# ftl/sdrainer

Measured on AMD Instinct MI355X. Metric: IQ MSamples/s through FFT+peak+envelope, higher is better.
Workload: dtype f64

## Files before the change

### sdrainer_amd/csrc/bank.h

```cpp
#pragma once
#include <hip/hip_runtime.h>

#include <algorithm>
#include <atomic>
#include <chrono>
#include <cmath>
#include <cstdio>
#include <cstdlib>
#include <cstring>
#include <memory>
#include <mutex>
#include <string>
#include <thread>
#include <vector>

#include "../../include/sdrainer_hip.h"
#include "host/delivery.h"
#include "host/frequency_mapping.h"
#include "sdr_device.h"

namespace sdrcapi {

inline thread_local std::string g_last_error;

// ... 70 lines not shown
    DevBuf<sdr::DevPeak> dev_peaks;
    DevBuf<int> peak_counts;
    hipEvent_t done[sdr::K_COUNT] = {};
    void release()
    {
        psd.release();
        tap.release();
        tapw.release();
        tap_used.release();
        fft_ctr.release();
        fft_scratch.release();
        win_mean.release();
        cum_part.release();
        recs.release();
        raw_bits.release();
        bits.release();
        edges.release();
        edge_counts.release();
        tr_values.release();
        tr_raw.release();
        tr_deb.release();
        slots_before.release();
        cum_out.release();
        dev_peaks.release();
        peak_counts.release();
        for (auto &e : done) {
            if (e)
                (void)hipEventDestroy(e);
            e = nullptr;
        }
    }
};


enum Parts { PART_SPECTRA = 1, PART_LISTEN = 2, PART_ALL = 3 };

struct CursorPack {
    sdr::BatchCursor c[RING];
};

}

struct sdr_bank {
    template <class T>
    using DevBuf = sdrcapi::DevBuf<T>;
    using BatchSet = sdrcapi::BatchSet;
    static constexpr int N_STAGES = sdrcapi::N_STAGES, GRAPH_PHASES = sdrcapi::GRAPH_PHASES, N_GRAPHS = sdrcapi::N_GRAPHS, RING = sdrcapi::RING;

    sdr_config cfg{};
    sdr::Switches sw;
    int logn = 0;
    int hop = 0;
    int device = 0;
    hipStream_t stream[N_STAGES] = {};
    bool own_stream[N_STAGES] = {};

    int max_chunks = 0;
    int text_cap = 2048;
    int edge_cap = 0;
    int bit_words = 0;

    DevBuf<fft64::cplx> tw;
    DevBuf<unsigned char> db_tab;
    DevBuf<int32_t> tap_bins;
    DevBuf<float> window;
    bool windowed = false;
    DevBuf<float> spectrum_row;
    std::vector<BatchSet> set;
    DevBuf<sdr::BandState> band_state;
    DevBuf<sdr::ListenerSlot> slots;
    DevBuf<uint16_t> morse;
    DevBuf<uint32_t> text;
    DevBuf<uint32_t> text_frames;
    DevBuf<uint32_t> edge_pos;
    DevBuf<float> carry[2];

    std::vector<sdr::BandState> h_band_state;
    std::vector<sdr::ListenerSlot> h_slots;
    std::vector<int> n_slots;
    std::vector<int64_t> center_frequency;
    int carry_cur = 0;
    int cum_count = 0;
    int64_t total_frames = 0;
    int64_t batch_index = 0;
    int last_set = 0, last_frames = 0, last_chunks = 0, last_count0 = 0;
    int last_carry_in = 0;
    int edge_width = 0;
    int find_peaks = 1;
    bool failed = false;
    DevBuf<sdr::DropCounters> drops;
    DevBuf<sdr::BatchCursor> cursors;
    hipGraph_t graph[GRAPH_PHASES][N_GRAPHS] = {};
    hipGraphExec_t graph_exec[GRAPH_PHASES][N_GRAPHS] = {};
    hipGraphNode_t graph_cursor_node[GRAPH_PHASES] = {};
    hipEvent_t phase_done[GRAPH_PHASES][N_GRAPHS] = {};
    int64_t graph_base = 0;
    int64_t graph_replays = 0;
    bool graph_ready = false;
    int graph_frames = 0, graph_slots = 0;
    sdr::InFormat graph_fmt = sdr::InFormat::F32;
    uint64_t attach_gen = 0, graph_attach_gen = 0;
    bool graph_results_on = false;
    int graph_find_peaks = 0;
    bool defer_listen = false, listen_pending = false;
    struct PendingListen {
        int set = 0, frames = 0;
// ... 91 lines not shown
```

### sdrainer_amd/csrc/capi_bank.hip

```cpp
#include "bank.h"
#include "twiddles.h"

using namespace sdrcapi;

namespace sdr {
int set_error(int code, const char *msg) { return fail(code, msg); }
}

namespace sdrcapi {
std::unique_ptr<host::DeliveryBackend> make_results_backend(sdr_bank *b);

void resolve_profile(sdr_bank *b)
{
    for (auto &p : b->pending) {
        float ms = 0.f;
        if (hipEventElapsedTime(&ms, p.second.first, p.second.second) == hipSuccess) {
            b->prof_ms[p.first] += ms;
            b->prof_n[p.first] += 1;
        }
        (void)hipEventDestroy(p.second.first);
        (void)hipEventDestroy(p.second.second);
    }
    b->pending.clear();
}
// ... 117 lines not shown
    return SDR_OK;
}

namespace {
static int self_check_once(int device_id)
{
    constexpr int kMax = 64;
    static std::mutex mu;
    static int verdict[kMax];
    static bool done[kMax];
    static std::string message[kMax];
    if (device_id < 0 || device_id >= kMax)
        return sdr_self_check(device_id);
    std::lock_guard<std::mutex> g(mu);
    if (!done[device_id]) {
        verdict[device_id] = sdr_self_check(device_id);
        message[device_id] = g_last_error;
        done[device_id] = verdict[device_id] == SDR_OK || message[device_id].find("self-check failed") != std::string::npos;
    }
    if (verdict[device_id] != SDR_OK)
        g_last_error = message[device_id];
    return verdict[device_id];
}
}

int sdr_create(const sdr_config *cfg, sdr_bank **out)
{
    if (!cfg || !out)
        return fail(SDR_ERR_BAD_ARG, "null argument");
    if (cfg->struct_size != (int32_t)sizeof(sdr_config))
        return fail(SDR_ERR_BAD_ARG, "sdr_config.struct_size mismatch (ABI)");
    const int N = cfg->block_size;
    if (N < 512 || N > 65536 || (N & (N - 1)))
        return fail(SDR_ERR_BAD_SIZE, "block_size must be a power of two in [512, 65536]");
    if (cfg->n_bands < 1 || cfg->sample_rate < 1 || cfg->max_batch_frames < 1 || cfg->max_listeners < 0 ||
        cfg->max_peaks < 1)
        return fail(SDR_ERR_BAD_ARG, "non-positive geometry");
    if (cfg->edge_width < 0 || N - 2 * cfg->edge_width < 10)
        return fail(SDR_ERR_BAD_ARG, "edge_width leaves fewer than 10 bins: the reference's windowSize would be 0 (NaN)");
    if (!sdr::hop_valid(cfg->hop, N))
        return fail(SDR_ERR_BAD_ARG, "hop must be 0 (= block_size) or a power of two with block_size / 16 <= hop <= block_size and hop >= 32");
    int ndev = 0;
    HIP_TRY(hipGetDeviceCount(&ndev));
    if (cfg->device_id < 0 || cfg->device_id >= ndev)
        return fail(SDR_ERR_BAD_ARG, "device_id out of range");
    HIP_TRY(hipSetDevice(cfg->device_id));

    sdr_bank *b = new sdr_bank();
    b->cfg = *cfg;
    b->hop = sdr::effective_hop(cfg->hop, N);
    b->sw = sdr::read_switches();
    b->device = cfg->device_id;
    b->logn = ilog2(N);
    b->edge_width = cfg->edge_width;
    b->find_peaks = cfg->find_peaks;
    const size_t B = (size_t)cfg->n_bands, L = (size_t)cfg->max_listeners;
    b->max_chunks = cfg->max_batch_frames / SDR_CUMULATION_SIZE + 2;
    b->edge_cap = cfg->max_batch_frames < 8192 ? cfg->max_batch_frames : 8192;
    b->bit_words = (cfg->max_batch_frames + 63) / 64;

#define ALLOC(buf, count)                                                                              \
    do {                                                                                               \
        hipError_t _e = (buf).alloc(count);                                                            \
        if (_e != hipSuccess) {                                                                        \
            sdr_destroy(b);                                                                            \
            return fail(SDR_ERR_HIP, std::string("hipMalloc " #buf ": ") + hipGetErrorString(_e));     \
        }                                                                                              \
    } while (0)

    for (int s = 1; s < N_STAGES && !b->sw.no_overlap; s++) {
        hipError_t e = hipStreamCreateWithFlags(&b->stream[s], hipStreamNonBlocking);
        if (e != hipSuccess) {
            sdr_destroy(b);
            return fail(SDR_ERR_HIP, "hipStreamCreate failed");
        }
        b->own_stream[s] = true;
    }
    if (sdr::may_use_matrix_pipe(b->sw, N)) {
        const int sc = self_check_once(cfg->device_id);
        if (sc != SDR_OK) {
            sdr_destroy(b);
            return sc;
        }
    }
    {
        std::vector<double> wre, wim;
        fft64::radix2_factors(N, wre, wim);
        const size_t ntw = (size_t)sdr::twiddle_count(b->logn);
        std::vector<fft64::cplx> h(ntw);
        sdr::build_twiddles(b->logn, wre.data(), wim.data(), h.data());
        ALLOC(b->tw, h.size());
        hipError_t e = hipMemcpy(b->tw.p, h.data(), h.size() * sizeof(fft64::cplx), hipMemcpyHostToDevice);
        std::vector<unsigned char> tab(gomath::kDbTabBytes);
        gomath::build_db_tables(b->logn, tab.data());
        ALLOC(b->db_tab, tab.size());
        if (e == hipSuccess)
            e = hipMemcpy(b->db_tab.p, tab.data(), tab.size(), hipMemcpyHostToDevice);
        if (e != hipSuccess) {
            sdr_destroy(b);
            return fail(SDR_ERR_HIP, "twiddle / table upload failed");
        }
    }
    b->res_backend = make_results_backend(b);
    b->results.reset(new host::Delivery(b->res_backend.get(), RING, GRAPH_PHASES * RING));
    b->set.reserve((size_t)RING + (size_t)GRAPH_PHASES * RING);
    b->set.resize(RING);
// ... 389 lines not shown
```

### sdrainer_amd/csrc/capi_process.hip

```cpp
#include <string>

#include "bank.h"

using namespace sdrcapi;

namespace sdrcapi {

constexpr int PUT_SLOTS = 16, PUT_BINS = 128;
struct SlotPack {
    int32_t n;
    int32_t index[PUT_SLOTS];
    sdr::ListenerSlot slot[PUT_SLOTS];
};
struct BinPack {
    int32_t n;
    int32_t index[PUT_BINS], bin[PUT_BINS];
};
__global__ void k_put_slots(sdr::ListenerSlot *slots, SlotPack p)
{
    constexpr int W = sizeof(sdr::ListenerSlot) / 4;
    static_assert(sizeof(sdr::ListenerSlot) % 4 == 0, "word copy");
    for (int i = threadIdx.x; i < p.n * W; i += blockDim.x)
        reinterpret_cast<uint32_t *>(slots + p.index[i / W])[i % W] = reinterpret_cast<const uint32_t *>(&p.slot[i / W])[i % W];
}
// ... 33 lines not shown
        HIP_TRY(hipGetLastError());
    }
    b->late_attached.clear();
    return SDR_OK;
}


int process_device_impl(sdr_bank *b, const void *iq_dev, int n_frames, size_t in_stride, sdr::InFormat fmt)
{
    if (b->failed)
        return fail(SDR_ERR_STATE, "an earlier process call failed half way; destroy the bank");
    if (b->graph_ready)
        return fail(SDR_ERR_STATE, "a graph is captured: process through sdr_graph_launch, or sdr_graph_release first");
    if (b->listen_pending)
        return fail(SDR_ERR_STATE, "the previous batch still waits for its listen half (sdr_process_listen)");
    const int rc = process_device_body(b, iq_dev, n_frames, in_stride, -1, -1, b->defer_listen ? PART_SPECTRA : PART_ALL, fmt);
    if (rc == SDR_ERR_HIP)
        b->failed = true;
    return rc;
}

int process_device_body(sdr_bank *b, const void *iq_dev, int n_frames, size_t in_stride, int capture_k, int capture_stage, int parts,
                        sdr::InFormat fmt)
{
    const bool cap = capture_k >= 0;
    const bool do_spectra = (parts & PART_SPECTRA) != 0, do_listen = (parts & PART_LISTEN) != 0;
    if (!do_spectra)
        n_frames = b->pend.frames;
    const sdr::BatchCursor *cur = cap ? b->cursors.p + capture_k : nullptr;
    const sdr_config &c = b->cfg;
    if (n_frames <= 0)
        return SDR_OK;
    struct DisarmOnExit {
        ~DisarmOnExit() { sdr::t_done_event = nullptr; }
    } disarm_on_exit;
    if (n_frames > c.max_batch_frames)
        return fail(SDR_ERR_BAD_ARG, "n_frames exceeds max_batch_frames");
    HIP_TRY(hipSetDevice(b->device));
    if (!cap) {
        const int frc = flush_late_attached(b);
        if (frc)
            return frc;
    }
    const int B = c.n_bands, N = c.block_size, stride = c.max_batch_frames;
    const sdr::NoiseGeom ng = b->noise_geom();
    const int si = cap ? RING + capture_k : do_spectra ? (int)(b->batch_index % RING) : b->pend.set;
    const int64_t first_frame = do_spectra ? b->total_frames : b->pend.first_frame;
    BatchSet &S = b->set[si];
    host::ResultSet &RS = b->results->set(si);
    int max_slots = 0;
    for (int i = 0; i < B; i++)
        max_slots = std::max(max_slots, b->n_slots[i]);
    const int count0 = b->cum_count;
    const sdr::BatchPlan P = sdr::plan_batch(b->sw, sdr::BatchGeometry{B, N, stride, b->max_chunks}, n_frames, count0, cap, max_slots, b->windowed);
    const int *plan = P.stream;
    const sdr::CumGeom cg{N, stride, n_frames, count0, b->max_chunks};
#define SDR_ON(k) (!cap || (capture_stage == G_THRESHOLDS ? (k) == sdr::K_THRESHOLDS : (plan[k] == capture_stage && (k) != sdr::K_THRESHOLDS)))
#if defined(SDR_DIAG)
#define SDR_LAUNCH(id, call) \
    do {                     \
        if (!(b->sw.diag_skip >> (id) & 1) && SDR_ON(id)) \
            HIP_TRY(call);   \
    } while (0)
#else
#define SDR_LAUNCH(id, call)  \
    do {                      \
        if (SDR_ON(id))       \
            HIP_TRY(call);    \
    } while (0)
#endif
    auto stream_of = [&](int k) { return b->stream[plan[k]]; };
    auto after = [&](int k, int dep) -> int {
        if (stream_of(k) != stream_of(dep) && !cap)
            HIP_TRY(hipStreamWaitEvent(stream_of(k), S.done[dep], 0));
        return SDR_OK;
    };
#define SDR_AFTER(k, dep)          \
    do {                           \
        int _rc = after((k), (dep)); \
        if (_rc)                   \
            return _rc;            \
    } while (0)
#define SDR_ARM(k) (sdr::t_done_event = cap ? nullptr : S.done[k])
#define SDR_DONE(k)                                                                                   \
    do {                                                                                              \
        if (sdr::t_done_event && !cap) {                                                              \
            sdr::t_done_event = nullptr;                                                              \
            HIP_TRY(hipEventRecord(S.done[k], stream_of(k)));                                         \
        }                                                                                             \
    } while (0)

    if (do_spectra) {
    if (b->results_on && !cap) {
        const int prc = b->results->park(si);
        if (prc)
            return prc;
    }
    {
        static const int launch_order[] = {sdr::K_WINDOW_MEANS, sdr::K_NOISE_STATS, sdr::K_THRESHOLDS, sdr::K_LISTEN_GATHER,
                                           sdr::K_LISTEN_DECODE, sdr::K_CUMULATE,   sdr::K_FIND_PEAKS};
        int last_on[N_STAGES];
        for (int &l : last_on)
            l = -1;
        for (int k : launch_order)
            last_on[plan[k]] = k;
        for (int st = 0; st < N_STAGES; st++) {
            const int k = last_on[st];
            if (k < 0 || st == plan[sdr::K_FFT])
                continue;
            if (cap)
                continue;
            if (hipEventQuery(S.done[k]) == hipSuccess)
                continue;
            HIP_TRY(hipStreamWaitEvent(stream_of(sdr::K_FFT), S.done[k], 0));
        }
    }
    if (cap && SDR_ON(sdr::K_FFT) && capture_k % RING == 0)
        HIP_TRY(launch_set_cursors(b->cursors.p + capture_k, CursorPack{}, stream_of(sdr::K_FFT)));
    {
        ProfScope ps(b, sdr::K_FFT, stream_of(sdr::K_FFT));
        SDR_ARM(sdr::K_FFT);
        sdr::FftTap tap{b->tap_bins.p, S.tap.p, max_slots, c.max_listeners};
        tap.wide = S.tapw.p;
        tap.used = S.tap_used.p;
        tap.steal = S.fft_ctr.p;
        tap.scratch = S.fft_scratch.p;
        tap.window = b->windowed ? b->window.p : nullptr;
        SDR_LAUNCH(sdr::K_FFT, sdr::launch_fft(b->logn, P.fft, fmt, iq_dev, cur, b->tw.p, S.psd.p, n_frames, B, in_stride, b->hop, stride, tap,
                                               stream_of(sdr::K_FFT)));
    }
    SDR_DONE(sdr::K_FFT);

    SDR_AFTER(sdr::K_WINDOW_MEANS, sdr::K_FFT);
    {
        ProfScope ps(b, sdr::K_WINDOW_MEANS, stream_of(sdr::K_WINDOW_MEANS));
        SDR_ARM(sdr::K_WINDOW_MEANS);
        if (P.noise_scan) {
            SDR_LAUNCH(sdr::K_WINDOW_MEANS, sdr::launch_psd_scan(S.psd.p, S.recs.p, S.cum_out.p, S.cum_part.p, cur, ng, cg, P.n_slots, B, P.bound_done,
                                                                 P.scan_parts, P.force_exact, stream_of(sdr::K_WINDOW_MEANS)));
        } else {
            SDR_LAUNCH(sdr::K_WINDOW_MEANS, sdr::launch_window_means(S.psd.p, S.win_mean.p, ng, n_frames, B, stride, P.wm_wpb,
                                                                     stream_of(sdr::K_WINDOW_MEANS)));
        }
    }
    SDR_DONE(sdr::K_WINDOW_MEANS);
    SDR_AFTER(sdr::K_NOISE_STATS, sdr::K_WINDOW_MEANS);
    {
        ProfScope ps(b, sdr::K_NOISE_STATS, stream_of(sdr::K_NOISE_STATS));
        SDR_ARM(sdr::K_NOISE_STATS);
        if (!P.noise_scan)
            SDR_LAUNCH(sdr::K_NOISE_STATS, sdr::launch_noise_stats(S.psd.p, S.win_mean.p, S.recs.p, ng, n_frames, B, stride, P.var_mfma,
                                                                   stream_of(sdr::K_NOISE_STATS)));
    }
    SDR_DONE(sdr::K_NOISE_STATS);
    SDR_AFTER(sdr::K_THRESHOLDS, sdr::K_NOISE_STATS);
    {
        ProfScope ps(b, sdr::K_THRESHOLDS, stream_of(sdr::K_THRESHOLDS));
        SDR_ARM(sdr::K_THRESHOLDS);
        SDR_LAUNCH(sdr::K_THRESHOLDS, sdr::launch_thresholds(S.recs.p, b->band_state.p, n_frames, B, stride,
                                                             stream_of(sdr::K_THRESHOLDS)));
    }
    SDR_DONE(sdr::K_THRESHOLDS);
    }

    sdr::ListenGeom lg;
    lg.n = N;
    lg.stride = stride;
    lg.max_listeners = c.max_listeners;
    lg.text_cap = b->text_cap;
    lg.edge_cap = b->edge_cap;
    lg.bit_words = b->bit_words;
    lg.trace = c.trace;
    lg.frame_base = (uint32_t)first_frame;
    if (do_listen) {
    SDR_AFTER(sdr::K_LISTEN_GATHER, sdr::K_THRESHOLDS);
    SDR_AFTER(sdr::K_LISTEN_GATHER, sdr::K_FFT);
    if (!cap && b->slots_put) {
        if (hipEventQuery(b->slots_put_ev) == hipSuccess)
            b->slots_put = false;
        else if (plan[sdr::K_LISTEN_GATHER] != S_LISTEN)
            HIP_TRY(hipStreamWaitEvent(stream_of(sdr::K_LISTEN_GATHER), b->slots_put_ev, 0));
    }
    SDR_ARM(sdr::K_LISTEN_GATHER);
    if (max_slots > 0) {
        ProfScope ps(b, sdr::K_LISTEN_GATHER, stream_of(sdr::K_LISTEN_GATHER));
        SDR_LAUNCH(sdr::K_LISTEN_GATHER, sdr::launch_listen_gather(S.tap.p, S.psd.p, S.recs.p, b->slots.p, b->db_tab.p, S.raw_bits.p, S.tr_values.p,
                                                                   S.tr_raw.p, cur, lg, n_frames, max_slots, B,
                                                                   stream_of(sdr::K_LISTEN_GATHER)));
    }
    SDR_DONE(sdr::K_LISTEN_GATHER);
    SDR_AFTER(sdr::K_LISTEN_DECODE, sdr::K_LISTEN_GATHER);
    if (c.trace && max_slots > 0 && SDR_ON(sdr::K_LISTEN_DECODE))
        HIP_TRY(hipMemcpyAsync(S.slots_before.p, b->slots.p, sizeof(sdr::ListenerSlot) * (size_t)B * (size_t)c.max_listeners,
                               hipMemcpyDeviceToDevice, stream_of(sdr::K_LISTEN_DECODE)));
    if (!b->results_on)
        SDR_ARM(sdr::K_LISTEN_DECODE);
    if (max_slots > 0) {
        ProfScope ps(b, sdr::K_LISTEN_DECODE, stream_of(sdr::K_LISTEN_DECODE));
        SDR_LAUNCH(sdr::K_LISTEN_DECODE, sdr::launch_listen_decode(b->slots.p, b->morse.p, S.raw_bits.p, S.bits.p, b->text.p,
                                                                   b->text_frames.p, S.edges.p, S.edge_counts.p, S.tr_deb.p, b->drops.p, cur,
                                                                   lg, n_frames, B, b->edge_pos.p, c.max_batch_frames, stream_of(sdr::K_LISTEN_DECODE)));
    }
    if (b->results_on && SDR_ON(sdr::K_LISTEN_DECODE)) {
        SDR_ARM(sdr::K_LISTEN_DECODE);
        HIP_TRY(sdr::launch_pack_listen(b->slots.p, S.edges.p, S.edge_counts.p, b->text.p, b->text_frames.p, b->drops.p, b->res_layout, max_slots, B,
                                        RS.block, stream_of(sdr::K_LISTEN_DECODE)));
        if (!cap)
            HIP_TRY(hipEventRecord(static_cast<hipEvent_t>(RS.ev_listen), stream_of(sdr::K_LISTEN_DECODE)));
    }
    SDR_DONE(sdr::K_LISTEN_DECODE);
    }
    if (!do_spectra) {
        b->results->complete(si, max_slots, b->pend.batch);
        b->listen_pending = false;
        return SDR_OK;
    }

    const int n_chunks = P.n_chunks;
    SDR_AFTER(sdr::K_CUMULATE, sdr::K_FFT);
    if (P.bound_done)
        SDR_AFTER(sdr::K_CUMULATE, sdr::K_WINDOW_MEANS);
    {
        ProfScope ps(b, sdr::K_CUMULATE, stream_of(sdr::K_CUMULATE));
        SDR_ARM(sdr::K_CUMULATE);
        SDR_LAUNCH(sdr::K_CUMULATE, sdr::launch_cumulate(S.psd.p, b->db_tab.p, b->carry[0].p, b->carry[1].p, b->carry_cur, S.cum_out.p, S.cum_part.p,
                                                         cur, cg, P.n_slots, B, P.bound, P.bound_done, P.scan_parts, stream_of(sdr::K_CUMULATE)));
    }
    SDR_DONE(sdr::K_CUMULATE);
    SDR_AFTER(sdr::K_FIND_PEAKS, sdr::K_CUMULATE);
    if (!b->results_on)
        SDR_ARM(sdr::K_FIND_PEAKS);
    if (b->find_peaks && n_chunks > 0) {
        SDR_AFTER(sdr::K_FIND_PEAKS, sdr::K_THRESHOLDS);
        ProfScope ps(b, sdr::K_FIND_PEAKS, stream_of(sdr::K_FIND_PEAKS));
        sdr::PeakGeom pg{N, stride, count0, b->max_chunks, c.max_peaks};
        sdr::FftTap wide_tap{nullptr, nullptr, max_slots, c.max_listeners};
        if (P.fft.wide_tap) {
            wide_tap.wide = S.tapw.p;
            wide_tap.used = S.tap_used.p;
        }
        SDR_LAUNCH(sdr::K_FIND_PEAKS, sdr::launch_find_peaks(S.cum_out.p, S.psd.p, b->db_tab.p, b->carry[0].p, b->carry[1].p, b->carry_cur, S.recs.p,
                                                             S.dev_peaks.p, S.peak_counts.p, cur, pg, n_frames, n_chunks, B, P.refine, wide_tap,
                                                             stream_of(sdr::K_FIND_PEAKS)));
    }
    if (b->results_on && SDR_ON(sdr::K_FIND_PEAKS)) {
        SDR_ARM(sdr::K_FIND_PEAKS);
        HIP_TRY(sdr::launch_pack_peaks(S.dev_peaks.p, S.peak_counts.p, cur, b->res_layout, b->find_peaks, n_frames, n_chunks, B,
                                       RS.block, stream_of(sdr::K_FIND_PEAKS)));
        if (!cap) {
            HIP_TRY(hipEventRecord(static_cast<hipEvent_t>(RS.ev_peaks), stream_of(sdr::K_FIND_PEAKS)));
            host::BatchMeta m;
            m.batch = b->batch_index;
            m.first_frame = b->total_frames;
            m.frames = n_frames;
            m.chunks = n_chunks;
            m.count0 = count0;
            m.slots = do_listen ? max_slots : 0;
            {
                std::lock_guard<std::mutex> guard(b->center_mu);
                m.center = b->center_frequency;
            }
            b->results->publish(si, std::move(m), do_listen);
        }
    }
    SDR_DONE(sdr::K_FIND_PEAKS);
#undef SDR_AFTER
#undef SDR_DONE
#undef SDR_ARM
#undef SDR_LAUNCH
#undef SDR_ON

    if (cap)
        return SDR_OK;
    b->last_carry_in = b->carry_cur;
    if (P.new_count != 0)
        b->carry_cur ^= 1;
    b->cum_count = P.new_count;
    b->last_set = si;
    b->last_frames = n_frames;
// ... 306 lines not shown
```

### sdrainer_amd/csrc/host/batch_plan.h

```cpp
#pragma once
#include <cstdint>
#include <cstdlib>
#include <cstring>

#include "../../../include/sdrainer_hip.h"

namespace sdr {

enum KernelId {
    K_FFT = 0, K_WINDOW_MEANS, K_NOISE_STATS, K_THRESHOLDS, K_LISTEN_GATHER, K_CUMULATE, K_FIND_PEAKS, K_LISTEN_DECODE,
    K_COUNT
};
enum Stage { S_FFT = 0, S_NOISE, S_LISTEN, S_PEAKS, N_STAGES };

constexpr int kR32MaxTap = 512;

struct Switches {
    bool noise_scan = true;
    int force_exact = 0;
    int fft_r32 = -1;
    int fft_fpw = 0;
    int cum_bound = -1;
    int refine_wide = -1;
    int var_mfma = -1;
    int wm_wpb = 0;
    int fft2p_group_mb = -1;
    bool no_overlap = false;
    bool graph_debug = false;
    int diag_skip = 0;
    int diag_plan[K_COUNT] = {-1, -1, -1, -1, -1, -1, -1, -1};
};

inline int tri_state(const char *e)
{
    if (!e)
        return -1;
    const int v = atoi(e);
    return v >= 0 ? (v != 0 ? 1 : 0) : -1;
}

inline Switches read_switches()
{
    Switches s;
    const char *e;
    if ((e = getenv("SDR_NOISE_PATH")))
        s.noise_scan = strcmp(e, "chains") != 0;
    if ((e = getenv("SDR_NOISE_FORCE_EXACT")))
        s.force_exact = atoi(e);
    if ((e = getenv("SDR_FFT_R32")))
        s.fft_r32 = atoi(e) ? 1 : 0;
    if ((e = getenv("SDR_FFT_FPW"))) {
        const int v = atoi(e);
        s.fft_fpw = v < 1 ? 1 : (v > 64 ? 64 : v);
    }
    s.cum_bound = tri_state(getenv("SDR_CUM_BOUND"));
    s.refine_wide = tri_state(getenv("SDR_REFINE_WIDE"));
    s.var_mfma = tri_state(getenv("SDR_VAR_MFMA"));
    if ((e = getenv("SDR_FFT2P_GROUP_MB")))
        s.fft2p_group_mb = atoi(e) >= 0 ? atoi(e) : -1;
    if ((e = getenv("SDR_WM_WPB")))
        s.wm_wpb = atoi(e) > 0 ? atoi(e) : 0;
    e = getenv("SDR_NO_OVERLAP");
    s.no_overlap = e && e[0] == '1';
    s.graph_debug = getenv("SDR_GRAPH_DEBUG") != nullptr;
#if defined(SDR_DIAG)
    if ((e = getenv("SDR_DIAG_SKIP")))
        s.diag_skip = atoi(e);
    if ((e = getenv("SDR_DIAG_PLAN")))
        for (int k = 0; k < K_COUNT && e[k] >= '0' && e[k] < '0' + N_STAGES; k++)
            s.diag_plan[k] = e[k] - '0';
#endif
    return s;
}

inline bool noise_scan_at(const Switches &sw, int n) { return sw.noise_scan && n <= 16384; }
inline bool var_mfma_at(const Switches &sw, int n, int n_frames)
{
    if (sw.var_mfma >= 0)
        return sw.var_mfma != 0;
    return n <= 16384 && n_frames < 4096;
}
inline bool may_use_matrix_pipe(const Switches &sw, int n) { return !noise_scan_at(sw, n) && (sw.var_mfma == 1 || (sw.var_mfma < 0 && n <= 16384)); }

struct FftChoice {
    bool r32 = false;
    int fpw = 0;
    bool wide_tap = false;
    bool two_phase = false;
    int group_frames = 0;
};

constexpr int kFft2pGroupMiB = 128;
inline int fft2p_group_frames(const Switches &sw, int n, int n_bands, int max_frames)
{
    if (n <= 16384 || n_bands <= 0 || max_frames <= 0)
        return 0;
    const int mib = sw.fft2p_group_mb >= 0 ? sw.fft2p_group_mb : kFft2pGroupMiB;
    const long per_frame = (long)n_bands * n * 16;
    const long f = mib == 0 ? max_frames : ((long)mib << 20) / per_frame;
    return (int)(f < 1 ? 1 : (f > max_frames ? max_frames : f));
}

inline FftChoice fft_choice(const Switches &sw, int n, int n_frames, int n_bands, int tap_n, bool windowed = false)
{
    FftChoice c;
    c.r32 = !windowed && n == 16384 && tap_n <= kR32MaxTap && (sw.fft_r32 == 1 || (sw.fft_r32 < 0 && (long)n_frames * n_bands >= 1024));
    c.fpw = sw.fft_fpw;
    c.wide_tap = c.r32 && tap_n > 0;
    c.two_phase = n > 16384;
    return c;
}

enum class Refine { NONE, NARROW, WIDE };

struct BatchGeometry {
    int n_bands, n, max_batch_frames, max_chunks;
};

struct BatchPlan {
    int stream[K_COUNT];
    FftChoice fft;
    bool noise_scan;
    int force_exact;
    bool var_mfma;
    int wm_wpb;
    bool bound;
    bool bound_done;
    int scan_parts;
    int n_slots;
    int n_chunks;
    int new_count;
    Refine refine;
};

inline BatchPlan plan_batch(const Switches &sw, const BatchGeometry &g, int n_frames, int count0, bool capturing, int max_slots,
                            bool windowed = false)
{
    BatchPlan p;
    const int plan[K_COUNT] = { S_FFT,         S_NOISE,  S_NOISE,  S_PEAKS,
                                S_LISTEN,   S_PEAKS,      S_PEAKS,   S_LISTEN};
    for (int k = 0; k < K_COUNT; k++)
        p.stream[k] = plan[k];
    if (!capturing && (long)g.n_bands * g.n <= 8192)
        p.stream[K_LISTEN_GATHER] = S_PEAKS;
    for (int k = 0; k < K_COUNT; k++)
        if (sw.diag_plan[k] >= 0)
            p.stream[k] = sw.diag_plan[k];

    p.fft = fft_choice(sw, g.n, n_frames, g.n_bands, max_slots, windowed);
    p.fft.group_frames = fft2p_group_frames(sw, g.n, g.n_bands, g.max_batch_frames);

    p.noise_scan = noise_scan_at(sw, g.n);
    p.force_exact = sw.force_exact;
    p.var_mfma = var_mfma_at(sw, g.n, n_frames);
    p.wm_wpb = sw.wm_wpb;

    p.bound = sw.cum_bound >= 0 ? sw.cum_bound != 0 : (double)n_frames * (double)g.n_bands * (double)g.n >= 64.0 * 1024.0 * 1024.0;
    p.bound_done = p.noise_scan && p.bound;

    p.n_chunks = (count0 + n_frames) / SDR_CUMULATION_SIZE;
    p.new_count = (count0 + n_frames) % SDR_CUMULATION_SIZE;
    p.n_slots = p.n_chunks + (p.new_count != 0 ? 1 : 0);
    if (capturing) {
        p.n_chunks = (SDR_CUMULATION_SIZE - 1 + n_frames) / SDR_CUMULATION_SIZE;
        p.n_slots = p.n_chunks + 1;
    }
    p.scan_parts = (long)p.n_slots * g.n_bands < 64 ? 2 : 1;

    const bool wide = sw.refine_wide >= 0 ? sw.refine_wide != 0 : (g.n >= 4096 && (long)p.n_chunks * g.n_bands >= 64);
    p.refine = !p.bound ? Refine::NONE : wide ? Refine::WIDE : Refine::NARROW;
    return p;
}

}
```

### sdrainer_amd/csrc/k_fft_psd.hip

```cpp
#include <hip/hip_runtime.h>

#include <algorithm>
#include <cstdlib>
#include <mutex>

#include "../../include/sdrainer_hip.h"
#include "cw_decoder.h"
#include "fft_f64.h"
#include "fft_r32.h"
#include "gomath.h"
#include "sc16.h"
#include "sdr_device.h"

#if !defined(SDR_FFT_WIN)
#define SDR_FFT_WIN 0
#endif
#if SDR_FFT_WIN
#define SDR_K_FFT_PSD k_fft_psd_win
#define SDR_K_FFT_PSD_SC16 k_fft_psd_sc16_win
#define SDR_WIN_PARAM , const float *__restrict__ win
#define SDR_WIN_ARG , win
#else
#define SDR_K_FFT_PSD k_fft_psd
#define SDR_K_FFT_PSD_SC16 k_fft_psd_sc16
// ... 896 lines not shown
        return hipGetLastError();
    }
    int fpw = fpw_asked > 0 ? fpw_asked : kDefaultFpw;
    while (fpw > 1 && (long)((n_frames + fpw - 1) / fpw) * n_bands < 256)
        fpw /= 2;
    if (fpw > 1)
        launch_kernel((SDR_K_FFT_PSD<LOGN, true>), dim3((n_frames + fpw - 1) / fpw, n_bands), dim3(PL::T), fft64::kLdsBytes<LOGN>, stream,
                           iq, cur, tw, psd, in_stride, frame_stride, out_stride, n_frames, fpw, tap.bins, tap.out, tap.n, tap.stride SDR_WIN_ARG);
    else
        launch_kernel((SDR_K_FFT_PSD<LOGN, false>), dim3(n_frames, n_bands), dim3(PL::T),
                           fft64::kLdsBytes<LOGN> + tap_lds + kPfSinkBytes, stream, iq, cur, tw, psd, in_stride,
                           frame_stride, out_stride, n_frames, 1, tap.bins, tap.out, tap.n, tap.stride SDR_WIN_ARG);
    return hipGetLastError();
    }
}

#if SDR_FFT_WIN
void window_layout(int logn, const float *w, float *out)
{
    switch (logn) {
    case 9: window_layout_t<9>(w, out); break;
    case 10: window_layout_t<10>(w, out); break;
    case 11: window_layout_t<11>(w, out); break;
    case 12: window_layout_t<12>(w, out); break;
    case 13: window_layout_t<13>(w, out); break;
    case 14: window_layout_t<14>(w, out); break;
    default:
        for (int i = 0; i < 1 << logn; i++)
            out[i] = w[i];
        break;
    }
}

hipError_t launch_fft_win(int logn, FftChoice fft, InFormat fmt, const void *iq, const BatchCursor *cur, const fft64::cplx *tw, float *psd,
                          int n_frames, int n_bands, size_t in_stride, int frame_stride, int out_stride, FftTap tap, hipStream_t stream)
{
    if (!tap.window || fft.r32 || fft.two_phase)
        return hipErrorInvalidValue;
#else
hipError_t launch_fft(int logn, FftChoice fft, InFormat fmt, const void *iq, const BatchCursor *cur, const fft64::cplx *tw, float *psd,
                      int n_frames, int n_bands, size_t in_stride, int frame_stride, int out_stride, FftTap tap, hipStream_t stream)
{
    if (fmt != InFormat::F32 && fmt != InFormat::SC16)
        return hipErrorInvalidValue;
    if (fft.two_phase)
        return launch_fft_2p(logn, fft, fmt, iq, cur, tw, psd, n_frames, n_bands, in_stride, frame_stride, out_stride, tap, stream);
    if (tap.window)
        return launch_fft_win(logn, fft, fmt, iq, cur, tw, psd, n_frames, n_bands, in_stride, frame_stride, out_stride, tap, stream);
    if (fft.r32) {
        if (logn != 14)
            return hipErrorInvalidValue;
        const fft64::cplx *tw32 = tw + fft64::Plan<14>::TW_TOTAL;
        if (fmt == InFormat::SC16)
            return launch_fft_r32_sc16(static_cast<const int16_t *>(iq), cur, tw32, psd, n_frames, n_bands, in_stride, frame_stride, out_stride, tap, stream);
        return launch_fft_r32(static_cast<const float *>(iq), cur, tw32, psd, n_frames, n_bands, in_stride, frame_stride, out_stride, tap, stream);
    }
#endif
    switch (logn) {
    case 9: return launch_fft_t<9>(fft.fpw, fmt, iq, cur, tw, psd, n_frames, n_bands, in_stride, frame_stride, out_stride, tap, stream);
    case 10: return launch_fft_t<10>(fft.fpw, fmt, iq, cur, tw, psd, n_frames, n_bands, in_stride, frame_stride, out_stride, tap, stream);
    case 11: return launch_fft_t<11>(fft.fpw, fmt, iq, cur, tw, psd, n_frames, n_bands, in_stride, frame_stride, out_stride, tap, stream);
    case 12: return launch_fft_t<12>(fft.fpw, fmt, iq, cur, tw, psd, n_frames, n_bands, in_stride, frame_stride, out_stride, tap, stream);
    case 13: return launch_fft_t<13>(fft.fpw, fmt, iq, cur, tw, psd, n_frames, n_bands, in_stride, frame_stride, out_stride, tap, stream);
    case 14: return launch_fft_t<14>(fft.fpw, fmt, iq, cur, tw, psd, n_frames, n_bands, in_stride, frame_stride, out_stride, tap, stream);
    default: return hipErrorInvalidValue;
    }
}
#if !SDR_FFT_WIN
hipError_t launch_fft(int logn, FftChoice fft, const float *iq, const BatchCursor *cur, const fft64::cplx *tw, float *psd, int n_frames,
                      int n_bands, size_t in_stride, int frame_stride, int out_stride, FftTap tap, hipStream_t stream)
{
    return launch_fft(logn, fft, InFormat::F32, iq, cur, tw, psd, n_frames, n_bands, in_stride, frame_stride, out_stride, tap, stream);
}

int twiddle_count(int logn)
{
    switch (logn) {
    case 9: return fft64::Plan<9>::TW_TOTAL;
    case 10: return fft64::Plan<10>::TW_TOTAL;
    case 11: return fft64::Plan<11>::TW_TOTAL;
    case 12: return fft64::Plan<12>::TW_TOTAL;
    case 13: return fft64::Plan<13>::TW_TOTAL;
    case 14: return fft64::Plan<14>::TW_TOTAL + r32_twiddle_count();
    case 15: return 1 << 14;
    case 16: return 1 << 15;
    default: return 0;
    }
}

void build_twiddles(int logn, const double *wre, const double *wim, fft64::cplx *out)
{
    switch (logn) {
    case 9: fft64::build_pass_twiddles<9>(wre, wim, out); break;
    case 10: fft64::build_pass_twiddles<10>(wre, wim, out); break;
    case 11: fft64::build_pass_twiddles<11>(wre, wim, out); break;
    case 12: fft64::build_pass_twiddles<12>(wre, wim, out); break;
    case 13: fft64::build_pass_twiddles<13>(wre, wim, out); break;
    case 14:
        fft64::build_pass_twiddles<14>(wre, wim, out);
        r32_build_twiddles(wre, wim, out + fft64::Plan<14>::TW_TOTAL);
        break;
    case 15:
    case 16:
        for (int i = 0; i < 1 << (logn - 1); i++)
            out[i] = fft64::cplx{wre[i], wim[i]};
        break;
    default: break;
    }
// ... 5 lines not shown
```

### sdrainer_amd/csrc/k_fft_r32.hip

```cpp
#include <hip/hip_runtime.h>

#include <algorithm>
#include <mutex>

#include "fft_r32.h"
#include "sdr_device.h"

#if !defined(SDR_R32_SC16)
#define SDR_R32_SC16 0
#endif
#if !defined(SDR_R32_HOP)
#define SDR_R32_HOP 0
#endif
#if SDR_R32_SC16
#include "sc16.h"
#define SDR_R32_IN int16_t
#else
#define SDR_R32_IN float
#endif
#if SDR_R32_HOP && SDR_R32_SC16
#define SDR_R32_KERNEL k_fft_r32_hop_sc16
#define SDR_R32_LAUNCH launch_fft_r32_hop_sc16
#elif SDR_R32_HOP
#define SDR_R32_KERNEL k_fft_r32_hop
// ... 437 lines not shown
        __syncthreads();
        SDR_R32_STAMP(st, RS_ROW);
        pf_point(PF_ROW);
        {
#pragma unroll
            for (int j = 0; j < N / 4 / T; j++)
                sv[j] = *reinterpret_cast<const u32x4 *>(smem + row_word(4 * (t + T * j)) * 4);
            const float *row = reinterpret_cast<const float *>(smem);
            const float tv = row[row_word(my_bin & (N - 1))];
            tapv = my_bin >= 0 ? tv : 0.0f;
            if (__builtin_amdgcn_readfirstlane(t) < n_tap && wide_b) {
                const rsrc_t wr = make_rsrc(wide_b + (size_t)frame * (4 * tap_stride), reg_tap ? (unsigned)tap_stride * 16u : 0u);
                u32x4 wv;
                wv.x = __float_as_uint(row[row_word((my_bin - 1) & (N - 1))]);
                wv.y = __float_as_uint(tv);
                wv.z = __float_as_uint(row[row_word((my_bin + 1) & (N - 1))]);
                wv.w = 0u;
                __builtin_amdgcn_raw_buffer_store_b128(wv, wr, t < n_tap ? (unsigned)t * 16u : 0x7ffffff0u, 0, 0);
            }
        }
        const unsigned after = __builtin_amdgcn_readfirstlane(claim_lds[0]);
        soft_arrive(soft + SOFT_ROW);
        SDR_R32_STAMP(st, RS_STORED);
#if defined(SDR_R32_PHASES)
        if (st.on && (threadIdx.x & 63) < RS_COUNT)
            g_r32_phases[threadIdx.x >> 6][threadIdx.x & 63] = st.v;
#endif
        prev = frame;
        frame = next;
        next = after;
        it++;
    }
    int t = tid;
    asm volatile("" : "+v"(t));
    flush_row(prev, t, 0, N / 4 / T);
    if (t == 0) {
        unsigned *const ctr = band_ctr();
        const unsigned done = __hip_atomic_fetch_add(ctr + 1, 1u, __ATOMIC_ACQ_REL, __HIP_MEMORY_SCOPE_AGENT);
        if (done == stash[2] - 1) {
            __hip_atomic_store(ctr, 0u, __ATOMIC_RELAXED, __HIP_MEMORY_SCOPE_AGENT);
            __hip_atomic_store(ctr + 1, 0u, __ATOMIC_RELAXED, __HIP_MEMORY_SCOPE_AGENT);
        }
    }
#endif
}

}

#if !SDR_R32_SC16 && !SDR_R32_HOP
int r32_twiddle_count() { return fft32::kTwTotal; }
void r32_build_twiddles(const double *wre, const double *wim, fft64::cplx *out) { fft32::build_twiddles(wre, wim, out); }
#endif

#if !defined(SDR_R32_RESERVE)
#define SDR_R32_RESERVE 0
#endif

hipError_t SDR_R32_LAUNCH(const SDR_R32_IN *iq, const BatchCursor *cur, const fft64::cplx *tw, float *psd, int n_frames, int n_bands,
                          size_t in_stride, int frame_stride, int out_stride, FftTap tap, hipStream_t stream)
{
    constexpr int kMaxDevices = 64;
    static std::once_flag setup_once[kMaxDevices];
    static hipError_t setup_err[kMaxDevices];
    static int cu_count[kMaxDevices];
    int dev = 0;
    hipError_t e = hipGetDevice(&dev);
    if (e != hipSuccess)
        return e;
    if (dev < 0 || dev >= kMaxDevices)
        return hipErrorInvalidDevice;
    std::call_once(setup_once[dev], [dev] {
        hipError_t se = hipFuncSetAttribute(reinterpret_cast<const void *>(&r32::SDR_R32_KERNEL), hipFuncAttributeMaxDynamicSharedMemorySize,
                                            r32::kLdsBytes);
        if (se == hipSuccess)
            se = hipDeviceGetAttribute(&cu_count[dev], hipDeviceAttributeMultiprocessorCount, dev);
        setup_err[dev] = se;
    });
    if (setup_err[dev] != hipSuccess)
        return setup_err[dev];
    if (n_frames <= 0 || n_bands <= 0)
        return hipSuccess;
    if (tap.n > fft32::T)
        return hipErrorInvalidValue;
    if (!tap.steal)
        return hipErrorInvalidValue;
    if (in_stride > 0xffffffffu)
        return hipErrorInvalidValue;
#if SDR_R32_HOP
    int shift = 0;
    while ((1 << shift) < frame_stride)
        shift++;
    if (frame_stride <= 0 || (1 << shift) != frame_stride || n_frames >= (1 << r32::kFrameBits))
        return hipErrorInvalidValue;
    const unsigned frames_and_shift = (unsigned)n_frames | (unsigned)shift << r32::kFrameBits;
#else
    if (frame_stride != fft32::N)
#if SDR_R32_SC16
        return launch_fft_r32_hop_sc16(iq, cur, tw, psd, n_frames, n_bands, in_stride, frame_stride, out_stride, tap, stream);
#else
        return launch_fft_r32_hop(iq, cur, tw, psd, n_frames, n_bands, in_stride, frame_stride, out_stride, tap, stream);
#endif
    const unsigned frames_and_shift = (unsigned)n_frames;
#endif
    const int cus = std::max(1, cu_count[dev] - SDR_R32_RESERVE);
    const int grid = std::min((cus + n_bands - 1) / n_bands, n_frames);
    launch_kernel(r32::SDR_R32_KERNEL, dim3(grid, n_bands), dim3(fft32::T), r32::kLdsBytes, stream, iq, cur, tw, psd, (unsigned)in_stride, out_stride,
                  frames_and_shift, tap.steal, tap.bins, tap.out, tap.n, tap.stride, tap.wide, tap.used);
    return hipGetLastError();
}

}
```

### sdrainer_amd/csrc/sdr_device.h

```cpp
#pragma once
#include <hip/hip_ext.h>
#include <hip/hip_runtime.h>

#include <cstdint>
#include <initializer_list>
#include <mutex>

#include "../../include/sdrainer_hip.h"
#include "cw_decoder.h"
#include "fft_f64.h"
#include "host/batch_plan.h"
#include "host/overlap.h"

namespace sdr {

struct BandState {
    float nf_ring[SDR_NOISE_WINDOW];
    float dev_ring[SDR_NOISE_WINDOW];
    float nf_sum, dev_sum;
    int32_t next;
    float peak_threshold;
};

struct ListenerSlot {
// ... 73 lines not shown
    if (done)
        hipExtLaunchKernelGGL(kernel, grid, block, lds_bytes, stream, nullptr, done, 0, args...);
    else
        hipLaunchKernelGGL(kernel, grid, block, lds_bytes, stream, args...);
}

struct LdsLimitOnce {
    static constexpr int kMaxDevices = 64;
    std::once_flag dev[kMaxDevices];
};
inline hipError_t raise_lds_limit_once(LdsLimitOnce &once, std::initializer_list<const void *> kernels, int bytes)
{
    int dev = 0;
    hipError_t e = hipGetDevice(&dev);
    if (e != hipSuccess)
        return e;
    if (dev < 0 || dev >= LdsLimitOnce::kMaxDevices)
        return hipErrorInvalidDevice;
    hipError_t attr_err = hipSuccess;
    std::call_once(once.dev[dev], [&] {
        for (const void *k : kernels) {
            const hipError_t ae = hipFuncSetAttribute(k, hipFuncAttributeMaxDynamicSharedMemorySize, bytes);
            if (ae != hipSuccess)
                attr_err = ae;
        }
    });
    return attr_err;
}

struct FftTap {
    const int32_t *bins;
    float *out;
    int n;
    int stride;
    float *wide = nullptr;
    int32_t *used = nullptr;
    uint32_t *steal = nullptr;
    fft64::cplx *scratch = nullptr;
    const float *window = nullptr;
};

hipError_t launch_fft(int logn, FftChoice fft, InFormat fmt, const void *iq, const BatchCursor *cur, const fft64::cplx *tw, float *psd,
                      int n_frames, int n_bands, size_t in_stride, int frame_stride, int out_stride, FftTap tap, hipStream_t stream);
hipError_t launch_fft(int logn, FftChoice fft, const float *iq, const BatchCursor *cur, const fft64::cplx *tw, float *psd, int n_frames,
                      int n_bands, size_t in_stride, int frame_stride, int out_stride, FftTap tap, hipStream_t stream);
hipError_t launch_fft_win(int logn, FftChoice fft, InFormat fmt, const void *iq, const BatchCursor *cur, const fft64::cplx *tw, float *psd,
                          int n_frames, int n_bands, size_t in_stride, int frame_stride, int out_stride, FftTap tap, hipStream_t stream);
void window_layout(int logn, const float *w, float *out);
hipError_t launch_fft_2p(int logn, FftChoice fft, InFormat fmt, const void *iq, const BatchCursor *cur, const fft64::cplx *tw, float *psd,
                         int n_frames, int n_bands, size_t in_stride, int frame_stride, int out_stride, FftTap tap, hipStream_t stream);
int twiddle_count(int logn);
void build_twiddles(int logn, const double *wre, const double *wim, fft64::cplx *out);
hipError_t launch_fft_r32(const float *iq, const BatchCursor *cur, const fft64::cplx *tw, float *psd, int n_frames, int n_bands,
                          size_t in_stride, int frame_stride, int out_stride, FftTap tap, hipStream_t stream);
hipError_t launch_fft_r32_sc16(const int16_t *iq, const BatchCursor *cur, const fft64::cplx *tw, float *psd, int n_frames, int n_bands,
                               size_t in_stride, int frame_stride, int out_stride, FftTap tap, hipStream_t stream);
hipError_t launch_fft_r32_hop(const float *iq, const BatchCursor *cur, const fft64::cplx *tw, float *psd, int n_frames, int n_bands,
                              size_t in_stride, int frame_stride, int out_stride, FftTap tap, hipStream_t stream);
hipError_t launch_fft_r32_hop_sc16(const int16_t *iq, const BatchCursor *cur, const fft64::cplx *tw, float *psd, int n_frames, int n_bands,
                                   size_t in_stride, int frame_stride, int out_stride, FftTap tap, hipStream_t stream);
int r32_twiddle_count();
void r32_build_twiddles(const double *wre, const double *wim, fft64::cplx *out);
hipError_t launch_window_means(const float *psd, double *win_mean, NoiseGeom g, int n_frames, int n_bands, int stride, int wpb_forced,
                               hipStream_t stream);
hipError_t launch_noise_stats(const float *psd, const double *win_mean, sdr_frame_rec *recs, NoiseGeom g, int n_frames,
                              int n_bands, int stride, bool mfma, hipStream_t stream);
hipError_t launch_mfma_order_probe(unsigned *mismatches, int order, hipStream_t stream);
hipError_t launch_thresholds(sdr_frame_rec *recs, BandState *st, int n_frames, int n_bands, int stride,
                             hipStream_t stream);
hipError_t launch_listen_gather(const float *tap, const float *psd, const sdr_frame_rec *recs, const ListenerSlot *slots, const void *db_tab,
                                uint64_t *raw_bits, float *tr_values, uint8_t *tr_raw, const BatchCursor *cur, ListenGeom g, int n_frames,
                                int n_slots, int n_bands, hipStream_t stream);
hipError_t launch_listen_decode(ListenerSlot *slots, const uint16_t *morse, const uint64_t *raw_bits,
                                uint64_t *deb_bits, uint32_t *text, uint32_t *text_frames, sdr_edge *edges,
                                uint32_t *edge_counts, uint8_t *tr_deb, DropCounters *drops, const BatchCursor *cur, ListenGeom g,
                                int n_frames, int n_bands, uint32_t *edge_pos, int pos_stride, hipStream_t stream);
hipError_t launch_listener_stop(ListenerSlot *slot, const uint16_t *morse, uint32_t *text, uint32_t *text_frames, int text_cap,
                                uint32_t frame, DropCounters *drops, hipStream_t stream);
hipError_t launch_set_debounce(ListenerSlot *slots, int n, int threshold, hipStream_t stream);
hipError_t launch_cumulate(const float *psd, const void *db_tab, float *carry0, float *carry1, int carry_in, float *cum_out,
                           const float *cum_part, const BatchCursor *cur, CumGeom g, int n_slots, int n_bands, bool bound, bool bound_done,
                           int parts, hipStream_t stream);
hipError_t launch_psd_scan(const float *psd, sdr_frame_rec *recs, float *cum_out, float *cum_part, const BatchCursor *cur, NoiseGeom ng,
                           CumGeom cg, int n_slots, int n_bands, bool do_bound, int parts, int force_exact, hipStream_t stream);
hipError_t launch_noise_exact_check(const float *psd_band, sdr_frame_rec *recs_band, NoiseGeom ng, int n_frames, unsigned *mismatches,
                                    hipStream_t stream);
hipError_t launch_spectrum_row(const float *psd_row, float *out, int n, hipStream_t stream);
hipError_t launch_pack_listen(ListenerSlot *slots, const sdr_edge *edges, const uint32_t *edge_counts, const uint32_t *text,
                              const uint32_t *text_frames, const DropCounters *drops, ResultsLayout lay, int n_slots, int n_bands, unsigned char *host,
                              hipStream_t stream);
hipError_t launch_pack_peaks(const DevPeak *peaks, const int *counts, const BatchCursor *cur, ResultsLayout lay, int find_peaks,
                             int n_frames, int n_chunks, int n_bands, unsigned char *host, hipStream_t stream);
__host__ __device__ inline int chunks_completed(int count0, int n_frames)
{
    const int first_len = SDR_CUMULATION_SIZE - count0;
    return n_frames >= first_len ? 1 + (n_frames - first_len) / SDR_CUMULATION_SIZE : 0;
}
hipError_t launch_unpack_be16(const uint8_t *raw, float *out, size_t n_values, hipStream_t stream);
hipError_t launch_unpack_sc16(const int16_t *raw, float *out, size_t n_values, hipStream_t stream);
hipError_t launch_find_peaks(float *cum, const float *psd, const void *db_tab, const float *carry0, const float *carry1, int carry_in,
                             const sdr_frame_rec *recs, DevPeak *peaks, int *counts, const BatchCursor *cur, PeakGeom g, int n_frames,
                             int n_chunks, int n_bands, Refine refine, FftTap tap, hipStream_t stream);
hipError_t launch_cumulation_row(const float *psd_band, const void *db_tab, const float *carry_in_band, float *row_out, CumGeom g, int slot,
                                 hipStream_t stream);

}
```

Before: 198,900.

## Reserve CUs from the r32 FFT grid so tail stages overlap on other streams

Queries the device CU count and, when the r32 FFT path runs with bounded cumulate and overlap enabled, shrinks the persistent FFT grid by up to a quarter of the CUs (at most 64). The freed CUs are meant to let the downstream scan and cumulate kernels on other streams run alongside the FFT instead of waiting for it. Diagnostic switches also allow moving the noise scan onto the FFT stream and changing how scan work is split. The trade-off is less FFT throughput when nothing overlaps with it.

After: 221,300, median of 4. +11.3%, better.

```diff
diff --git a/sdrainer_amd/csrc/bank.h b/sdrainer_amd/csrc/bank.h
--- a/sdrainer_amd/csrc/bank.h
+++ b/sdrainer_amd/csrc/bank.h
@@ -146,6 +146,7 @@
     int logn = 0;
     int hop = 0;
     int device = 0;
+    int n_cus = 0;
     hipStream_t stream[N_STAGES] = {};
     bool own_stream[N_STAGES] = {};
 
diff --git a/sdrainer_amd/csrc/capi_bank.hip b/sdrainer_amd/csrc/capi_bank.hip
--- a/sdrainer_amd/csrc/capi_bank.hip
+++ b/sdrainer_amd/csrc/capi_bank.hip
@@ -193,6 +193,8 @@
     b->sw = sdr::read_switches();
     b->device = cfg->device_id;
     b->logn = ilog2(N);
+    if (hipDeviceGetAttribute(&b->n_cus, hipDeviceAttributeMultiprocessorCount, cfg->device_id) != hipSuccess || b->n_cus < 0)
+        b->n_cus = 0;
     b->edge_width = cfg->edge_width;
     b->find_peaks = cfg->find_peaks;
     const size_t B = (size_t)cfg->n_bands, L = (size_t)cfg->max_listeners;
diff --git a/sdrainer_amd/csrc/capi_process.hip b/sdrainer_amd/csrc/capi_process.hip
--- a/sdrainer_amd/csrc/capi_process.hip
+++ b/sdrainer_amd/csrc/capi_process.hip
@@ -109,8 +109,11 @@
     for (int i = 0; i < B; i++)
         max_slots = std::max(max_slots, b->n_slots[i]);
     const int count0 = b->cum_count;
-    const sdr::BatchPlan P = sdr::plan_batch(b->sw, sdr::BatchGeometry{B, N, stride, b->max_chunks}, n_frames, count0, cap, max_slots, b->windowed);
-    const int *plan = P.stream;
+    const sdr::BatchPlan P = sdr::plan_batch(b->sw, sdr::BatchGeometry{B, N, stride, b->max_chunks, b->n_cus}, n_frames, count0, cap, max_slots,
+                                             b->windowed);
+    int plan[sdr::K_COUNT];
+    for (int k = 0; k < sdr::K_COUNT; k++)
+        plan[k] = sdr::stage_of(P, k);
     const sdr::CumGeom cg{N, stride, n_frames, count0, b->max_chunks};
 #define SDR_ON(k) (!cap || (capture_stage == G_THRESHOLDS ? (k) == sdr::K_THRESHOLDS : (plan[k] == capture_stage && (k) != sdr::K_THRESHOLDS)))
 #if defined(SDR_DIAG)
@@ -194,23 +197,26 @@
         SDR_ARM(sdr::K_WINDOW_MEANS);
         if (P.noise_scan) {
             SDR_LAUNCH(sdr::K_WINDOW_MEANS, sdr::launch_psd_scan(S.psd.p, S.recs.p, S.cum_out.p, S.cum_part.p, cur, ng, cg, P.n_slots, B, P.bound_done,
-                                                                 P.scan_parts, P.force_exact, stream_of(sdr::K_WINDOW_MEANS)));
+                                                                 P.scan_deal, P.force_exact, stream_of(sdr::K_WINDOW_MEANS)));
         } else {
             SDR_LAUNCH(sdr::K_WINDOW_MEANS, sdr::launch_window_means(S.psd.p, S.win_mean.p, ng, n_frames, B, stride, P.wm_wpb,
                                                                      stream_of(sdr::K_WINDOW_MEANS)));
         }
     }
     SDR_DONE(sdr::K_WINDOW_MEANS);
-    SDR_AFTER(sdr::K_NOISE_STATS, sdr::K_WINDOW_MEANS);
-    {
-        ProfScope ps(b, sdr::K_NOISE_STATS, stream_of(sdr::K_NOISE_STATS));
-        SDR_ARM(sdr::K_NOISE_STATS);
-        if (!P.noise_scan)
-            SDR_LAUNCH(sdr::K_NOISE_STATS, sdr::launch_noise_stats(S.psd.p, S.win_mean.p, S.recs.p, ng, n_frames, B, stride, P.var_mfma,
-                                                                   stream_of(sdr::K_NOISE_STATS)));
-    }
-    SDR_DONE(sdr::K_NOISE_STATS);
-    SDR_AFTER(sdr::K_THRESHOLDS, sdr::K_NOISE_STATS);
+    const int noise_done = P.scan_behind_fft ? sdr::K_WINDOW_MEANS : sdr::K_NOISE_STATS;
+    if (!P.scan_behind_fft) {
+        SDR_AFTER(sdr::K_NOISE_STATS, sdr::K_WINDOW_MEANS);
+        {
+            ProfScope ps(b, sdr::K_NOISE_STATS, stream_of(sdr::K_NOISE_STATS));
+            SDR_ARM(sdr::K_NOISE_STATS);
+            if (!P.noise_scan)
+                SDR_LAUNCH(sdr::K_NOISE_STATS, sdr::launch_noise_stats(S.psd.p, S.win_mean.p, S.recs.p, ng, n_frames, B, stride, P.var_mfma,
+                                                                       stream_of(sdr::K_NOISE_STATS)));
+        }
+        SDR_DONE(sdr::K_NOISE_STATS);
+    }
+    SDR_AFTER(sdr::K_THRESHOLDS, noise_done);
     {
         ProfScope ps(b, sdr::K_THRESHOLDS, stream_of(sdr::K_THRESHOLDS));
         SDR_ARM(sdr::K_THRESHOLDS);
@@ -281,7 +287,7 @@
         ProfScope ps(b, sdr::K_CUMULATE, stream_of(sdr::K_CUMULATE));
         SDR_ARM(sdr::K_CUMULATE);
         SDR_LAUNCH(sdr::K_CUMULATE, sdr::launch_cumulate(S.psd.p, b->db_tab.p, b->carry[0].p, b->carry[1].p, b->carry_cur, S.cum_out.p, S.cum_part.p,
-                                                         cur, cg, P.n_slots, B, P.bound, P.bound_done, P.scan_parts, stream_of(sdr::K_CUMULATE)));
+                                                         cur, cg, P.n_slots, B, P.bound, P.bound_done, P.scan_deal, stream_of(sdr::K_CUMULATE)));
     }
     SDR_DONE(sdr::K_CUMULATE);
     SDR_AFTER(sdr::K_FIND_PEAKS, sdr::K_CUMULATE);
diff --git a/sdrainer_amd/csrc/host/batch_plan.h b/sdrainer_amd/csrc/host/batch_plan.h
--- a/sdrainer_amd/csrc/host/batch_plan.h
+++ b/sdrainer_amd/csrc/host/batch_plan.h
@@ -29,6 +29,7 @@
     bool graph_debug = false;
     int diag_skip = 0;
     int diag_plan[K_COUNT] = {-1, -1, -1, -1, -1, -1, -1, -1};
+    int diag_tail[3] = {-1, -1, -1};
 };
 
 inline int tri_state(const char *e)
@@ -69,6 +70,12 @@
     if ((e = getenv("SDR_DIAG_PLAN")))
         for (int k = 0; k < K_COUNT && e[k] >= '0' && e[k] < '0' + N_STAGES; k++)
             s.diag_plan[k] = e[k] - '0';
+    if ((e = getenv("SDR_DIAG_TAIL")))
+        for (int i = 0; i < 3 && e && *e; i++) {
+            s.diag_tail[i] = atoi(e) >= 0 ? atoi(e) : -1;
+            e = strchr(e, ',');
+            e = e ? e + 1 : e;
+        }
 #endif
     return s;
 }
@@ -88,6 +95,7 @@
     bool wide_tap = false;
     bool two_phase = false;
     int group_frames = 0;
+    int reserve_cus = 0;
 };
 
 constexpr int kFft2pGroupMiB = 128;
@@ -115,6 +123,7 @@
 
 struct BatchGeometry {
     int n_bands, n, max_batch_frames, max_chunks;
+    int n_cus = 0;
 };
 
 struct BatchPlan {
@@ -131,7 +140,17 @@
     int n_chunks;
     int new_count;
     Refine refine;
-};
+    bool scan_behind_fft;
+    int scan_deal;
+};
+
+inline int stage_of(const BatchPlan &p, int k)
+{
+    return p.scan_behind_fft && (k == K_WINDOW_MEANS || k == K_NOISE_STATS) ? p.stream[K_FFT] : p.stream[k];
+}
+
+constexpr int kTailReserveCus = 64;
+inline int tail_reserve_cus(int n_cus) { return n_cus / 4 < kTailReserveCus ? n_cus / 4 : kTailReserveCus; }
 
 inline BatchPlan plan_batch(const Switches &sw, const BatchGeometry &g, int n_frames, int count0, bool capturing, int max_slots,
                             bool windowed = false)
@@ -169,6 +188,19 @@
 
     const bool wide = sw.refine_wide >= 0 ? sw.refine_wide != 0 : (g.n >= 4096 && (long)p.n_chunks * g.n_bands >= 64);
     p.refine = !p.bound ? Refine::NONE : wide ? Refine::WIDE : Refine::NARROW;
+
+    const bool tail = g.n_cus > 0 && p.fft.r32 && p.bound_done && !capturing && !sw.no_overlap;
+    p.fft.reserve_cus = tail ? tail_reserve_cus(g.n_cus) : 0;
+    p.scan_behind_fft = false;
+    p.scan_deal = p.scan_parts;
+    if (p.fft.r32 && p.noise_scan && !capturing && !sw.no_overlap) {
+        if (sw.diag_tail[0] >= 0)
+            p.fft.reserve_cus = g.n_cus > 0 && sw.diag_tail[0] >= g.n_cus ? g.n_cus - 1 : sw.diag_tail[0];
+        if (sw.diag_tail[1] >= 0 && p.bound_done)
+            p.scan_deal = sw.diag_tail[1] >= 2 ? 2 : 1;
+        if (sw.diag_tail[2] >= 0)
+            p.scan_behind_fft = sw.diag_tail[2] != 0;
+    }
     return p;
 }
 
diff --git a/sdrainer_amd/csrc/k_fft_psd.hip b/sdrainer_amd/csrc/k_fft_psd.hip
--- a/sdrainer_amd/csrc/k_fft_psd.hip
+++ b/sdrainer_amd/csrc/k_fft_psd.hip
@@ -972,8 +972,8 @@
             return hipErrorInvalidValue;
         const fft64::cplx *tw32 = tw + fft64::Plan<14>::TW_TOTAL;
         if (fmt == InFormat::SC16)
-            return launch_fft_r32_sc16(static_cast<const int16_t *>(iq), cur, tw32, psd, n_frames, n_bands, in_stride, frame_stride, out_stride, tap, stream);
-        return launch_fft_r32(static_cast<const float *>(iq), cur, tw32, psd, n_frames, n_bands, in_stride, frame_stride, out_stride, tap, stream);
+            return launch_fft_r32_sc16(static_cast<const int16_t *>(iq), cur, tw32, psd, n_frames, n_bands, in_stride, frame_stride, out_stride, tap, fft.reserve_cus, stream);
+        return launch_fft_r32(static_cast<const float *>(iq), cur, tw32, psd, n_frames, n_bands, in_stride, frame_stride, out_stride, tap, fft.reserve_cus, stream);
     }
 #endif
     switch (logn) {
diff --git a/sdrainer_amd/csrc/k_fft_r32.hip b/sdrainer_amd/csrc/k_fft_r32.hip
--- a/sdrainer_amd/csrc/k_fft_r32.hip
+++ b/sdrainer_amd/csrc/k_fft_r32.hip
@@ -513,12 +513,8 @@
 void r32_build_twiddles(const double *wre, const double *wim, fft64::cplx *out) { fft32::build_twiddles(wre, wim, out); }
 #endif
 
-#if !defined(SDR_R32_RESERVE)
-#define SDR_R32_RESERVE 0
-#endif
-
 hipError_t SDR_R32_LAUNCH(const SDR_R32_IN *iq, const BatchCursor *cur, const fft64::cplx *tw, float *psd, int n_frames, int n_bands,
-                          size_t in_stride, int frame_stride, int out_stride, FftTap tap, hipStream_t stream)
+                          size_t in_stride, int frame_stride, int out_stride, FftTap tap, int reserve_cus, hipStream_t stream)
 {
     constexpr int kMaxDevices = 64;
     static std::once_flag setup_once[kMaxDevices];
@@ -557,13 +553,13 @@
 #else
     if (frame_stride != fft32::N)
 #if SDR_R32_SC16
-        return launch_fft_r32_hop_sc16(iq, cur, tw, psd, n_frames, n_bands, in_stride, frame_stride, out_stride, tap, stream);
-#else
-        return launch_fft_r32_hop(iq, cur, tw, psd, n_frames, n_bands, in_stride, frame_stride, out_stride, tap, stream);
+        return launch_fft_r32_hop_sc16(iq, cur, tw, psd, n_frames, n_bands, in_stride, frame_stride, out_stride, tap, reserve_cus, stream);
+#else
+        return launch_fft_r32_hop(iq, cur, tw, psd, n_frames, n_bands, in_stride, frame_stride, out_stride, tap, reserve_cus, stream);
 #endif
     const unsigned frames_and_shift = (unsigned)n_frames;
 #endif
-    const int cus = std::max(1, cu_count[dev] - SDR_R32_RESERVE);
+    const int cus = std::max(1, cu_count[dev] - std::max(reserve_cus, 0));
     const int grid = std::min((cus + n_bands - 1) / n_bands, n_frames);
     launch_kernel(r32::SDR_R32_KERNEL, dim3(grid, n_bands), dim3(fft32::T), r32::kLdsBytes, stream, iq, cur, tw, psd, (unsigned)in_stride, out_stride,
                   frames_and_shift, tap.steal, tap.bins, tap.out, tap.n, tap.stride, tap.wide, tap.used);
diff --git a/sdrainer_amd/csrc/sdr_device.h b/sdrainer_amd/csrc/sdr_device.h
--- a/sdrainer_amd/csrc/sdr_device.h
+++ b/sdrainer_amd/csrc/sdr_device.h
@@ -149,13 +149,13 @@
 int twiddle_count(int logn);
 void build_twiddles(int logn, const double *wre, const double *wim, fft64::cplx *out);
 hipError_t launch_fft_r32(const float *iq, const BatchCursor *cur, const fft64::cplx *tw, float *psd, int n_frames, int n_bands,
-                          size_t in_stride, int frame_stride, int out_stride, FftTap tap, hipStream_t stream);
+                          size_t in_stride, int frame_stride, int out_stride, FftTap tap, int reserve_cus, hipStream_t stream);
 hipError_t launch_fft_r32_sc16(const int16_t *iq, const BatchCursor *cur, const fft64::cplx *tw, float *psd, int n_frames, int n_bands,
-                               size_t in_stride, int frame_stride, int out_stride, FftTap tap, hipStream_t stream);
+                               size_t in_stride, int frame_stride, int out_stride, FftTap tap, int reserve_cus, hipStream_t stream);
 hipError_t launch_fft_r32_hop(const float *iq, const BatchCursor *cur, const fft64::cplx *tw, float *psd, int n_frames, int n_bands,
-                              size_t in_stride, int frame_stride, int out_stride, FftTap tap, hipStream_t stream);
+                              size_t in_stride, int frame_stride, int out_stride, FftTap tap, int reserve_cus, hipStream_t stream);
 hipError_t launch_fft_r32_hop_sc16(const int16_t *iq, const BatchCursor *cur, const fft64::cplx *tw, float *psd, int n_frames, int n_bands,
-                                   size_t in_stride, int frame_stride, int out_stride, FftTap tap, hipStream_t stream);
+                                   size_t in_stride, int frame_stride, int out_stride, FftTap tap, int reserve_cus, hipStream_t stream);
 int r32_twiddle_count();
 void r32_build_twiddles(const double *wre, const double *wim, fft64::cplx *out);
 hipError_t launch_window_means(const float *psd, double *win_mean, NoiseGeom g, int n_frames, int n_bands, int stride, int wpb_forced,
```
